# weibohuang0314/pixel_aware_gyro_aided_klt_feature_tracker

Measured on AMD Instinct MI355X. Metric: tracked features/sec (21x21, 3-lvl, 30 iter), higher is better.
Workload: dtype f32 sampling, f64 normal equations; 1 GPU; cfg1_euroc_752x480: 752x480 pair, 1000 keypoints (1000/GPU), gyro-predicted affine init, h=10, L=3, I=30 (synthetic stand-in for BASELINE configs[1]); mode=shard-weak, features_total=1000, features_active=1000, step_mode=graph

## Files before the change

### pixel_aware_gyro_aided_klt_feature_tracker_amd/csrc/pagk_device.h

```cpp
#pragma once
#include <hip/hip_runtime.h>
#include <stdint.h>

namespace pagk {

constexpr int kMaxLevels = 8;

struct DevLevel {
    const uint32_t *quad;
    int cols, rows;
    float fcols, frows;
    float fcols_m1, frows_m1;
};

__device__ __forceinline__ int ld_agent(const int *p) { return __hip_atomic_load(p, __ATOMIC_RELAXED, __HIP_MEMORY_SCOPE_AGENT); }
__device__ __forceinline__ void st_agent(int *p, int v) { __hip_atomic_store(p, v, __ATOMIC_RELAXED, __HIP_MEMORY_SCOPE_AGENT); }

struct SuspState {
    int level;
    int iter;
    float dx, dy, dg, db, lastCost;
    int iters;
};

// ... 481 lines not shown
                                                      uint32_t sv, OperandRange &rg)
{
    const double H00 = M[0][0], H10 = M[1][0], H11 = M[1][1], H20 = M[2][0], H21 = M[2][1], H22 = M[2][2];
    const double H30 = M[3][0], H31 = M[3][1], H32 = M[3][2], H33 = M[3][3];
    const bool recip = (sv & SV_LLT_RECIP) != 0;
    auto scale = [&](double n, const Den &D, double rx) { return recip ? n * rx : div_by<FAST>(n, D, rg); };
    const bool ok0 = FAST || (!(H00 <= 0.0));
    const double d0 = pivot_root_early<FAST>(ok0, H00, H00, rg);
    const Den D0 = den_prepare<FAST>(d0, rg);
    double rx = recip ? div_by<FAST>(1.0, D0, rg) : 0.0;
    const double q10 = scale(H10, D0, rx), q20 = scale(H20, D0, rx), q30 = scale(H30, D0, rx);
    const double r0 = div_by<FAST>(b[0], D0, rg);
    const double L10 = ok0 ? q10 : H10, L20 = ok0 ? q20 : H20, L30 = ok0 ? q30 : H30;
    const double x1 = H11 - L10 * L10;
    const bool ok1 = FAST || (ok0 && !(x1 <= 0.0));
    const double d1 = pivot_root_early<FAST>(ok1, x1, H11, rg);
    const Den D1 = den_prepare<FAST>(d1, rg);
    rx = recip ? div_by<FAST>(1.0, D1, rg) : 0.0;
    const double q21 = scale(H21 - L20 * L10, D1, rx), q31 = scale(H31 - L30 * L10, D1, rx);
    const double r1 = div_by<FAST>(b[1] - L10 * r0, D1, rg);
    const double L21 = ok1 ? q21 : H21, L31 = ok1 ? q31 : H31;
    double s = L20 * L20;
    s += L21 * L21;
    const double x2 = H22 - s;
    const bool ok2 = FAST || (ok1 && !(x2 <= 0.0));
    const double d2 = pivot_root_early<FAST>(ok2, x2, H22, rg);
    const Den D2 = den_prepare<FAST>(d2, rg);
    s = L30 * L20;
    s += L31 * L21;
    rx = recip ? div_by<FAST>(1.0, D2, rg) : 0.0;
    const double q32 = scale(H32 - s, D2, rx);
    const double r2 = div_by<FAST>(b[2] - (L20 * r0 + L21 * r1), D2, rg);
    const double L32 = ok2 ? q32 : H32;
    const double a0 = L30 * L30, a1 = L31 * L31, a2 = L32 * L32;
    const double x3 = H33 - ((sv & SV_PIVOT_TREE) ? a0 + (a1 + a2) : (a0 + a1) + a2);
    const bool ok3 = ok2 && !(x3 <= 0.0);
    const double d3 = pivot_root<FAST>(ok3, x3, H33, rg);
    const Den D3 = den_prepare<FAST>(d3, rg);
    const double c0 = L30 * r0, c1 = L31 * r1, c2 = L32 * r2;
    const double r3 = div_by<FAST, true>(b[3] - ((sv & SV_LOWER_SEQ) ? (c0 + c1) + c2 : c0 + (c1 + c2)), D3, rg);
    return llt4_upper_nsq<FAST>(r0, r1, r2, r3, L10, L20, L21, L30, L31, L32, D0, D1, D2, D3, sv, x, rg);
}

__device__ __forceinline__ double llt4_solve_nsq(const double (&M)[4][4], const double (&b)[4], double (&x)[4],
                                                 uint32_t sv)
{
    OperandRange rg;
    double nsq = llt4_solve_nsq_form<true>(M, b, x, sv, rg);
    if (!rg.in_range()) nsq = llt4_solve_nsq_form<false>(M, b, x, sv, rg);
    return nsq;
}

__device__ __forceinline__ double llt4_solve_norm(const double (&M)[4][4], const double (&b)[4], double (&x)[4],
                                                  uint32_t sv)
{
    OperandRange rg;
    return sqrt(llt4_solve_nsq_form<false>(M, b, x, sv, rg));
}

__device__ __forceinline__ double lane_bcast(double v, int src)
{
    int lo = __double2loint(v), hi = __double2hiint(v);
    lo = __builtin_amdgcn_readlane(lo, src);
    hi = __builtin_amdgcn_readlane(hi, src);
    return __hiloint2double(hi, lo);
}
template <int K>
__device__ __forceinline__ double row_bcast(double v)
{
    return __builtin_amdgcn_update_dpp(0.0, v, 0x150 + K, 0xf, 0xf, false);
}

#ifdef PAGK_COUNT_REDO
static __device__ uint32_t g_redo_lo, g_redo_hi;
#endif
template <int K, bool ROWB>
__device__ __forceinline__ double solve_bcast(double v)
{
    if constexpr (ROWB)
        return row_bcast<K>(v);
    else
        return lane_bcast(v, K);
}
template <bool FAST, bool ROWB = false>
__device__ __forceinline__ double llt4_solve_nsq_lanes_form(const double (&M)[4][4], const double (&b)[4], int l,
                                                            double (&x)[4], uint32_t sv, OperandRange &rg)
{
    const double H00 = M[0][0], H10 = M[1][0], H11 = M[1][1], H20 = M[2][0], H21 = M[2][1], H22 = M[2][2];
    const double H30 = M[3][0], H31 = M[3][1], H32 = M[3][2], H33 = M[3][3];
    const bool recip = (sv & SV_LLT_RECIP) != 0;
    auto column = [&](double n, const Den &D, bool fwd) {
        const double q = div_by<FAST>(n, D, rg);
        if (!recip) return q;
        const double rx = div_by<FAST>(1.0, D, rg);
        return fwd ? q : n * rx;
    };
    const bool ok0 = FAST || (!(H00 <= 0.0));
    const double d0 = pivot_root_early<FAST>(ok0, H00, H00, rg);
    const Den D0 = den_prepare<FAST>(d0, rg);
    const double n0 = l == 0 ? b[0] : (l == 1 ? H10 : (l == 2 ? H20 : H30));
    const double q0 = column(n0, D0, l == 0);
    const double own0 = (l == 0 || ok0) ? q0 : n0;
    double r0 = solve_bcast<0, ROWB>(own0);
    const double L10 = solve_bcast<1, ROWB>(own0), L20 = solve_bcast<2, ROWB>(own0), L30 = solve_bcast<3, ROWB>(own0);
    const double x1 = H11 - L10 * L10;
    const bool ok1 = FAST || (ok0 && !(x1 <= 0.0));
    const double d1 = pivot_root_early<FAST>(ok1, x1, H11, rg);
    const Den D1 = den_prepare<FAST>(d1, rg);
    const double h1 = l == 2 ? H21 : H31;
    const double n1 = l == 1 ? b[1] - L10 * r0 : h1 - (l == 2 ? L20 : L30) * L10;
    const double q1 = column(n1, D1, l == 1);
    const double own1 = (l == 1 || ok1) ? q1 : h1;
    double r1 = solve_bcast<1, ROWB>(own1);
    const double L21 = solve_bcast<2, ROWB>(own1), L31 = solve_bcast<3, ROWB>(own1);
    double s = L20 * L20;
    s += L21 * L21;
    const double x2 = H22 - s;
    const bool ok2 = FAST || (ok1 && !(x2 <= 0.0));
    const double d2 = pivot_root_early<FAST>(ok2, x2, H22, rg);
    const Den D2 = den_prepare<FAST>(d2, rg);
    s = L30 * L20;
    s += L31 * L21;
    const double n2 = l == 2 ? b[2] - (L20 * r0 + L21 * r1) : H32 - s;
    const double q2 = column(n2, D2, l == 2);
    const double own2 = (l == 2 || ok2) ? q2 : H32;
    double r2 = solve_bcast<2, ROWB>(own2);
    const double L32 = solve_bcast<3, ROWB>(own2);
    const double a0 = L30 * L30, a1 = L31 * L31, a2 = L32 * L32;
    const double x3 = H33 - ((sv & SV_PIVOT_TREE) ? a0 + (a1 + a2) : (a0 + a1) + a2);
    const bool ok3 = ok2 && !(x3 <= 0.0);
    const double d3 = pivot_root<FAST>(ok3, x3, H33, rg);
    const Den D3 = den_prepare<FAST>(d3, rg);
    const double c0 = L30 * r0, c1 = L31 * r1, c2 = L32 * r2;
    const double r3 = div_by<FAST, true>(b[3] - ((sv & SV_LOWER_SEQ) ? (c0 + c1) + c2 : c0 + (c1 + c2)), D3, rg);
    return llt4_upper_nsq<FAST>(r0, r1, r2, r3, L10, L20, L21, L30, L31, L32, D0, D1, D2, D3, sv, x, rg);
}

template <bool ROWB = false>
__device__ __forceinline__ double llt4_solve_nsq_lanes(const double (&M)[4][4], const double (&b)[4], int l,
                                                       double (&x)[4], uint32_t sv)
{
    OperandRange rg;
    double nsq = llt4_solve_nsq_lanes_form<true, ROWB>(M, b, l, x, sv, rg);
#ifndef PAGK_EXPERIMENT_NO_REDO
    if (__builtin_amdgcn_ballot_w64(!rg.in_range() && l < 4) != 0) nsq = llt4_solve_nsq_lanes_form<false, ROWB>(M, b, l, x, sv, rg);
#endif
#ifdef PAGK_COUNT_REDO
    g_redo_lo = rg.t;
#endif
    return nsq;
}

__device__ __forceinline__ double repeat_sum_f64(double q, int P)
{
    if (!(q > 0.0)) return (double)P * q;
    double x = 32.0 * q;
    int k = 32;
    double top = __hiloint2double((__double2hiint(q) & 0x7ff00000) + (6 << 20), 0);
    double M = 0.75 * top;
#pragma unroll
    for (int b = 0; b < 5; b++) {
        const double I = (q + M) - M;
        const float est = (float)(top - x) * __builtin_amdgcn_rcpf((float)I);
        int n = (int)est - 1;
        const int lim = (P - k) - 4 * (5 - b);
        n = n > lim ? lim : n;
        n = n < 0 ? 0 : n;
        x = __builtin_fma((double)n, I, x);
        k += n + 4;
        x = x + q;
        x = x + q;
        x = x + q;
        x = x + q;
        M *= 2.0;
        top *= 2.0;
    }
    return x;
}

__device__ __forceinline__ double add_penalty_hb(const TrackArgs &a, float dx, float dy, double (&H)[4][4],
                                                 double (&b)[4])
{
    double d = (double)sqrtf(dx * dx + dy * dy);
    double e_pen = (double)a.lam_invlog * soft_log((double)a.alpha * d + 1);
    double jx = (double)a.lam_invlog_alpha / ((double)a.alpha * d + 1) * ((double)dx / d);
    double jy = (double)a.lam_invlog_alpha / ((double)a.alpha * d + 1) * ((double)dy / d);
    H[0][0] += jx * jx;
    H[1][0] += jy * jx;
    H[1][1] += jy * jy;
    H[2][0] += 0.0 * jx;
    H[2][1] += 0.0 * jy;
    H[2][2] += 0.0 * 0.0;
    H[3][0] += 0.0 * jx;
    H[3][1] += 0.0 * jy;
    H[3][2] += 0.0 * 0.0;
    H[3][3] += 0.0 * 0.0;
    b[0] += jx * e_pen;
    b[1] += jy * e_pen;
    b[2] += 0.0 * e_pen;
    b[3] += 0.0 * e_pen;
    return e_pen * e_pen;
}
__device__ __forceinline__ void add_penalty(const TrackArgs &a, float dx, float dy, double (&H)[4][4],
                                            double (&b)[4], float &cost)
{
    const double epsq = add_penalty_hb(a, dx, dy, H, b);
    cost = (float)((double)cost + epsq);
}

__device__ __forceinline__ void distort_point(const TrackArgs &a, float ux, float uy, float &ox, float &oy)
{
    if (!a.distort_on) {
        ox = ux;
        oy = uy;
        return;
    }
    float x = (ux - a.cx) * a.fx_inv;
    float y = (uy - a.cy) * a.fy_inv;
    float r2 = x * x + y * y;
    float r4 = r2 * r2;
    float r6 = r4 * r2;
    float xd = x * (1 + a.k1 * r2 + a.k2 * r4 + a.k3 * r6) + 2 * a.p1 * x * y + a.p2 * (r2 + 2 * x * x);
    float yd = y * (1 + a.k1 * r2 + a.k2 * r4 + a.k3 * r6) + a.p1 * (r2 + 2 * y * y) + 2 * a.p2 * x * y;
    ox = a.fx * xd + a.cx;
    oy = a.fy * yd + a.cy;
}
// ... 3 lines not shown
```

### pixel_aware_gyro_aided_klt_feature_tracker_amd/csrc/pagk_hip.hip

```cpp
#include <hip/hip_runtime.h>

#include <cmath>
#include <cstdio>
#include <cstdlib>
#include <cstring>
#include <new>
#include <vector>

#include "../../include/pagk.h"
#include "pagk_kernels.h"

using namespace pagk;

namespace {

constexpr int kSlots = 6;
constexpr int kUserSlots = 4;

struct FrameSlot {
    int w = 0, h = 0, L = 0;
    int wrap0 = 1;
    int pad0 = 0;
    uint8_t *u8[kMaxLevels] = {};
    uint32_t *quad[kMaxLevels] = {};
// ... 288 lines not shown
{
    int lw[kMaxLevels], lh[kMaxLevels];
    level_dims(s.w, s.h, s.L, lw, lh);
    bool all_even = s.L <= 4;
    for (int l = 0; l + 1 < s.L; l++) all_even = all_even && !(lw[l] & 1) && !(lh[l] & 1);
    return all_even;
}

int slot_build(pagk_ctx *ctx, FrameSlot &s, const uint8_t *src0, int64_t pitch0, int wrap0)
{
    s.pad0 = wrap0 ? 0 : 2;
    int lw[kMaxLevels], lh[kMaxLevels];
    level_dims(s.w, s.h, s.L, lw, lh);
    dim3 blk(32, 8);
    if (ctx->ev_pyr[0] && !in_capture(ctx)) HIPCHK(ctx, hipEventRecord(ctx->ev_pyr[0], ctx->stream));
    bool all_even = true;
    for (int l = 0; l + 1 < s.L; l++) all_even = all_even && !(lw[l] & 1) && !(lh[l] & 1);
    if (s.L <= 4 && !ctx->unfused_pyramid && all_even) {
        PyrArgs pa;
        const int nb = make_pyr_args(s, src0, pitch0, wrap0, &pa);
        hipLaunchKernelGGL(k_pyramid_fused, dim3(nb), dim3(256), 0, ctx->stream, pa);
        HIPCHK(ctx, hipGetLastError());
        if (ctx->ev_pyr[1] && !in_capture(ctx)) HIPCHK(ctx, hipEventRecord(ctx->ev_pyr[1], ctx->stream));
        if (!in_capture(ctx)) ctx->pyr_timed = true;
        s.wrap0 = wrap0;
        s.valid = true;
        return PAGK_OK;
    }
    const uint8_t *src = src0;
    int64_t pitch = pitch0;
    for (int l = 0; l < s.L; l++) {
        if (l > 0) {
            dim3 grd((lw[l] + 31) / 32, (lh[l] + 7) / 8);
            if (!(lw[l - 1] & 1) && !(lh[l - 1] & 1))
                hipLaunchKernelGGL(k_pyr_down, grd, blk, 0, ctx->stream, src, pitch, lw[l], lh[l], s.u8[l]);
            else
                hipLaunchKernelGGL(k_pyr_down_linear, grd, blk, 0, ctx->stream, src, pitch, lw[l - 1], lh[l - 1], lw[l],
                                   lh[l], 1. / ((double)lw[l] / lw[l - 1]), 1. / ((double)lh[l] / lh[l - 1]), s.u8[l]);
            src = s.u8[l];
            pitch = lw[l];
        }
        dim3 grd((lw[l] + 31) / 32, (lh[l] + 7) / 8);
        hipLaunchKernelGGL(k_build_quads, grd, blk, 0, ctx->stream, src, pitch, lw[l], lh[l], l == 0 ? wrap0 : 1,
                           s.quad[l]);
    }
    HIPCHK(ctx, hipGetLastError());
    if (ctx->ev_pyr[1] && !in_capture(ctx)) HIPCHK(ctx, hipEventRecord(ctx->ev_pyr[1], ctx->stream));
    if (!in_capture(ctx)) ctx->pyr_timed = true;
    s.wrap0 = wrap0;
    s.valid = true;
    return PAGK_OK;
}

int check_params(const pagk_params *p)
{
    if (!p) return PAGK_E_ARG;
    if (p->half_patch < 1 || p->half_patch > PAGK_MAX_HALF_PATCH) return PAGK_E_ARG;
    if (p->iterations < 0 || p->pyramids < 1 || p->pyramids > PAGK_MAX_PYRAMIDS) return PAGK_E_ARG;
    if (p->inverse) return PAGK_E_UNSUPPORTED;
    if (p->solver_variant & ~(SV_LOWER_SEQ | SV_UPPER_TREE | SV_NORM_SEQ | SV_LLT_RECIP | SV_PIVOT_TREE)) return PAGK_E_ARG;
    return PAGK_OK;
}

void fill_level(DevLevel &d, const FrameSlot &s, int l)
{
    int w = s.w, h = s.h;
    for (int k = 0; k < l; k++) {
        w = (int)(w * 0.5);
        h = (int)(h * 0.5);
    }
    d.quad = s.quad[l];
    d.cols = w;
    d.rows = h;
    d.fcols = (float)w;
    d.frows = (float)h;
    d.fcols_m1 = (float)(w - 1);
    d.frows_m1 = (float)(h - 1);
}

int lv_check(pagk_ctx *ctx)
{
    if (ctx->lv_error && *static_cast<volatile int *>(ctx->lv_error) != 0) {
        *static_cast<volatile int *>(ctx->lv_error) = 0;
        snprintf(ctx->err, sizeof(ctx->err), "a wave of the level-by-level tracking launch gave up waiting for the level above");
        return PAGK_E_HIP;
    }
    return PAGK_OK;
}

int no_live_graphs(pagk_ctx *ctx, const char *what)
{
    for (int k = 0; k < pagk_ctx::kGraphs; k++)
        if (ctx->graph_execs[k]) {
            snprintf(ctx->err, sizeof(ctx->err), "%s would have to grow while graph %d of this context is alive (its nodes hold the old "
                     "pointers): destroy the graph first, or run the largest launch once before capturing", what, k);
            return PAGK_E_ARG;
        }
    return PAGK_OK;
}

int quad_capacity(pagk_ctx *ctx, int half)
{
    const int slot = half == 5 ? 0 : (half == 7 ? 1 : 2);
    if (ctx->quad_capacity[slot] == 0) {
        int per_cu = 0;
        hipError_t e = half == 5   ? hipOccupancyMaxActiveBlocksPerMultiprocessor(&per_cu, k_track_quad<2>, 64, 0)
                       : half == 7 ? hipOccupancyMaxActiveBlocksPerMultiprocessor(&per_cu, k_track_quad<4>, 64, 0)
                                   : hipOccupancyMaxActiveBlocksPerMultiprocessor(&per_cu, k_track_quad<7>, 64, 0);
        if (e != hipSuccess || per_cu <= 0) per_cu = 16;
        ctx->quad_capacity[slot] = per_cu * (ctx->cus > 0 ? ctx->cus : 256);
    }
    return ctx->quad_capacity[slot];
}

int quad_budget_for(pagk_ctx *ctx, int waves, int iterations, int levels, int half)
{
    if (ctx->quad_budget >= 0) return ctx->quad_budget;
    if (iterations * levels < 60) return 0;
    const long long cap = quad_capacity(ctx, half);
    const bool exposed_tail = 100ll * waves > 45 * cap && 100ll * waves <= 125 * cap;
    if (ctx->concurrency != 1 || !exposed_tail || (in_capture(ctx) && !ctx->capturing)) return 0;
    return 20;
}

int levels_budget_for(pagk_ctx *ctx, int quads, int iterations, int levels, int half, bool *live)
{
    const bool foreign = in_capture(ctx) && !ctx->capturing;
    *live = !foreign || ctx->quad_budget >= 0;
    if (ctx->quad_budget >= 0) return ctx->quad_budget;
    if (iterations * levels < 60 || ctx->concurrency != 1) return 0;
    const long long cap = quad_capacity(ctx, half);
    if (100ll * quads <= 45 * cap) return 0;
    if (foreign && 100ll * quads > 125 * cap) return 0;
    return 20;
}

void fill_param_args(TrackArgs &a, const pagk_params *p)
{
    a.half = p->half_patch;
    a.iterations = p->iterations;
    a.has_gyro = p->has_gyro_predict_initial;
    a.illum = p->consider_illumination;
    a.use_affine = p->consider_affine;
    a.penalty = p->regularization_penalty;
    a.calc_ncc = p->calculate_ncc;
    a.solver = p->solver_variant;
    float invlog = p->inv_log_max_dist != 0.0f ? p->inv_log_max_dist
                                               : pagk_inv_log_max_dist(p->alpha, p->max_distance);
    a.lam_invlog = p->lambda * invlog;
    a.lam_invlog_alpha = a.lam_invlog * p->alpha;
    a.alpha = p->alpha;
    a.win_size_inv = (double)(1.0f / (2.0f * p->half_patch + 1.0f) / (2.0f * p->half_patch + 1.0f));
    a.distort_on = p->dist_coef[0] != 0.0f;
    a.fx = p->fx, a.fy = p->fy, a.cx = p->cx, a.cy = p->cy;
    a.fx_inv = (float)(1.0 / (double)p->fx);
    a.fy_inv = (float)(1.0 / (double)p->fy);
    a.k1 = p->dist_coef[0], a.k2 = p->dist_coef[1], a.p1 = p->dist_coef[2], a.p2 = p->dist_coef[3];
    a.k3 = p->n_dist_coef == 5 ? p->dist_coef[4] : 0.0f;
}

int launch_track(pagk_ctx *ctx, const pagk_params *p, const FrameSlot &sr, const FrameSlot &sc, int n,
                 const float *d_pt_ref, const float *d_pt_init, const float *d_affine, const uint8_t *d_status,
                 const pagk_outputs *o, const PyrArgs *pyr = nullptr, int pyr_blocks = 0, bool *pyr_done = nullptr)
{
    if (pyr_done) *pyr_done = false;
    TrackArgs a;
    memset(&a, 0, sizeof a);
    a.n_levels = p->pyramids;
    for (int l = 0; l < p->pyramids; l++) {
        fill_level(a.l1[l], sr, l);
        fill_level(a.l2[l], sc, l);
        a.scales[l] = l == 0 ? 1.0f : (float)((double)a.scales[l - 1] * 0.5);
    }
    a.n = n;
    a.pt_ref = d_pt_ref;
    a.pt_init = d_pt_init;
    a.affine = d_affine;
    a.status_in = d_status;
    a.pt_un = o->pt_un;
    a.pt_dist = o->pt_dist;
    a.status = o->status;
    a.pix_err = o->pix_err;
    a.dist_pred = o->dist_pred;
    a.ncc = o->ncc;
    a.iters = o->iters;
#if defined(PAGK_STAMPS) || defined(PAGK_COUNT_REDO) || defined(PAGK_TIC)
    a.dbg = reinterpret_cast<unsigned long long *>(getenv("PAGK_DBG_PTR") ? strtoull(getenv("PAGK_DBG_PTR"), nullptr, 0) : 0ull);
#endif
    fill_param_args(a, p);
    a.prio_k = ctx->prio_k;
    a.prio_stats = ctx->prio_stats;
    a.prio_kbuf = ctx->prio_stats ? reinterpret_cast<const int *>(ctx->prio_stats + 2) : nullptr;

    if (ctx->ev_trk[0] && !in_capture(ctx)) HIPCHK(ctx, hipEventRecord(ctx->ev_trk[0], ctx->stream));
    if (n > 0) {
        const int Pm = (2 * a.half + 1) * (2 * a.half + 1);
        const bool mfma_ok = a.half == 5 || a.half == 7 || a.half == 10;
        ctx->last_handover = false;
        const bool lean = !a.penalty && a.solver == 0;
        const long long n_sel = (long long)n * ctx->concurrency;
#ifdef PAGK_ALL_VARIANTS
        const bool use_rows = mfma_ok && !a.calc_ncc && a.iterations >= 1 && ctx->kernel == 6;
#else
        const bool use_rows = false;
#endif
        const bool use_levels = mfma_ok && !a.calc_ncc && p->pyramids >= 2 && ctx->lv_error &&
                                (ctx->kernel == 7 || (ctx->kernel == 0 && (ctx->concurrency == 1 || ctx->levels_shared) &&
                                                      n_sel >= ctx->levels_min_features));
        const bool quad_like = ctx->kernel == 5 || ctx->kernel == 6 || ctx->kernel == 7;
        const bool use_quad = !use_rows && !use_levels && mfma_ok && !a.calc_ncc && (quad_like || (ctx->kernel == 0 && n_sel >= ctx->quad_min_features));
        const bool use_wave = !use_quad && !use_rows && !use_levels && mfma_ok && (ctx->kernel == 3 || quad_like || (ctx->kernel == 0 && n_sel >= ctx->wave_min_features));
#ifdef PAGK_ALL_VARIANTS
        const bool use_mfma = !use_wave && mfma_ok && (ctx->kernel == 2 || (ctx->kernel == 0 && n_sel >= ctx->mfma_min_features));
#else
        const bool use_mfma = false;
#endif
        ctx->last_variant = ctx->kernel == 1 ? 1 : use_levels ? 7 : use_rows ? 6 : (use_quad ? 5 : (use_wave ? 3 : ((ctx->kernel == 4 && mfma_ok) ? 4 : (use_mfma ? 2 : 0))));
        if (ctx->kernel == 1) {
            hipLaunchKernelGGL(k_track_thread, dim3((n + 63) / 64), dim3(64), 0, ctx->stream, a);
#ifdef PAGK_ALL_VARIANTS
        } else if (use_rows) {
            const int nch = (Pm + 63) / 64;
            const int slot = a.half == 5 ? 0 : (a.half == 7 ? 1 : 2);
            if (ctx->rows_capacity[slot] == 0) {
                int per_cu = 0, cus = 0;
                hipError_t oe = a.half == 5   ? hipOccupancyMaxActiveBlocksPerMultiprocessor(&per_cu, k_track_rows<2>, 64, 0)
                                : a.half == 7 ? hipOccupancyMaxActiveBlocksPerMultiprocessor(&per_cu, k_track_rows<4>, 64, 0)
                                              : hipOccupancyMaxActiveBlocksPerMultiprocessor(&per_cu, k_track_rows<7>, 64, 0);
                HIPCHK(ctx, oe);
                HIPCHK(ctx, hipDeviceGetAttribute(&cus, hipDeviceAttributeMultiprocessorCount, ctx->device));
                ctx->rows_capacity[slot] = per_cu * cus > 0 ? per_cu * cus : 1024;
            }
            int waves = (n + 3) / 4 < ctx->rows_capacity[slot] ? (n + 3) / 4 : ctx->rows_capacity[slot];
            if (ctx->rows_waves_cap > 0 && waves > ctx->rows_waves_cap) waves = ctx->rows_waves_cap;
            const size_t need = (size_t)waves * 4 * nch * 64 * sizeof(float);
            if (need > ctx->quad_ws_bytes) {
                if (in_capture(ctx)) {
                    snprintf(ctx->err, sizeof(ctx->err), "the row kernel's workspace would have to be (re)allocated during graph capture");
                    return PAGK_E_ARG;
                }
                if (int gr = no_live_graphs(ctx, "the row kernel's workspace")) return gr;
                if (ctx->quad_ws) HIPCHK(ctx, hipFree(ctx->quad_ws));
                ctx->quad_ws = nullptr;
                ctx->quad_ws_bytes = 0;
                HIPCHK(ctx, hipMalloc(&ctx->quad_ws, need));
                ctx->quad_ws_bytes = need;
            }
            a.ws = static_cast<float *>(ctx->quad_ws);
            a.queue = static_cast<int *>(ctx->queue);
            HIPCHK(ctx, hipMemsetAsync(a.queue, 0, 4, ctx->stream));
            auto launch = [&](auto kern) -> hipError_t {
                hipLaunchKernelGGL(kern, dim3(waves), dim3(64), 0, ctx->stream, a);
                return hipGetLastError();
            };
            hipError_t e = hipErrorInvalidValue;
            if (a.half == 5) e = launch(k_track_rows<2>);
            else if (a.half == 7) e = launch(k_track_rows<4>);
            else if (a.half == 10) e = launch(k_track_rows<7>);
            HIPCHK(ctx, e);
#endif
        } else if (use_quad || use_levels) {
            const int nch = (Pm + 63) / 64, nq = (n + 3) / 4, waves = use_levels ? nq * p->pyramids : nq;
            const size_t need = (size_t)waves * 4 * nch * 64 * sizeof(float);
            const size_t ready_bytes = use_levels ? align_up((size_t)(p->pyramids - 1) * 8 * ((nq + 7) / 8) * 4, 256) : 0;
            const size_t susp_zero = 256 + align_up((size_t)n * 4, 256);
            const size_t need_lv = use_levels ? 32768 + ready_bytes + susp_zero + (size_t)n * 16 + (size_t)n * sizeof(SuspState) : 0;
            if (need > ctx->quad_ws_bytes || need_lv > ctx->lv_bytes) {
                if (in_capture(ctx)) {
                    snprintf(ctx->err, sizeof(ctx->err), "the quad kernel's workspace would have to be (re)allocated during graph capture");
                    return PAGK_E_ARG;
                }
                if (int gr = no_live_graphs(ctx, "the quad kernel's workspace")) return gr;
                if (need > ctx->quad_ws_bytes) {
                    if (ctx->quad_ws) HIPCHK(ctx, hipFree(ctx->quad_ws));
                    ctx->quad_ws = nullptr;
// ... 1623 lines not shown
```

### pixel_aware_gyro_aided_klt_feature_tracker_amd/csrc/pagk_pipe_kernel.h

```cpp
#pragma once

namespace pagk {


__device__ __forceinline__ bool lds_wait_ge(const int *flag, int want)
{
    for (uint32_t look = 0; look < kPipeWaitLooks; look++) {
        if (__builtin_amdgcn_readfirstlane(*reinterpret_cast<const volatile int *>(flag)) >= want) return true;
        __builtin_amdgcn_s_sleep(1);
    }
    return false;
}

__device__ __forceinline__ void lds_store_b32(uint32_t addr, int v)
{
    asm volatile("ds_write_b32 %0, %1" ::"v"(addr), "v"(v) : "memory");
}

template <int H, bool LEAN>
__device__ __forceinline__ void track_pipe_body(const TrackArgs &a, const int i, const SuspState *resume = nullptr)
{
    static_assert(H >= 8 && H <= 10, "two-round patches only");
    constexpr int kBlock = 256;
    constexpr int Wd = 2 * H + 1, P = Wd * Wd, PP = (P + 31) / 32 * 32, PS = PP + 1;
    constexpr int TAIL = P % 32;
    constexpr bool HAS_B = P > 320, HAS_C = P > 384;
    extern __shared__ __attribute__((aligned(16))) unsigned char lds_raw[];
    const int tid = threadIdx.x;
    const int wave = __builtin_amdgcn_readfirstlane(tid >> 6), lane = tid & 63;

    double *stream = reinterpret_cast<double *>(lds_raw);
    float *esq = reinterpret_cast<float *>(stream + (size_t)8 * PS);
    double *cslot = reinterpret_cast<double *>(esq + PP);
    double *acc = cslot + 2;
    double *sh_upd = acc + 16;
    float *sh_cost = reinterpret_cast<float *>(sh_upd + 5);
    int *flags = reinterpret_cast<int *>(sh_cost + 2 + 2);
    double *h22 = reinterpret_cast<double *>(flags + 4);
    double *sh_pen = h22 + 2;

    const float *init = a.has_gyro ? a.pt_init : a.pt_ref;
    float p2x = init[2 * i], p2y = init[2 * i + 1];
    if (!a.status_in[i]) {
        if (tid == 0) write_outputs(a, i, p2x, p2y, 0, 0.0f, 0, 0.0f, 0);
        return;
    }
    float A00 = 1, A01 = 0, A10 = 0, A11 = 1;
    if (a.use_affine) {
        A00 = a.affine[4 * i], A01 = a.affine[4 * i + 1], A10 = a.affine[4 * i + 2], A11 = a.affine[4 * i + 3];
    }
    const float refx = a.pt_ref[2 * i], refy = a.pt_ref[2 * i + 1];
    if (tid < 4) flags[tid] = 0;

    int pix[3];
    pix[0] = tid;
    pix[1] = (wave == 3 ? 320 : 256) + lane;
    pix[2] = 384 + lane;
    float px[3], py[3], wx[3], wy[3];
#pragma unroll
    for (int r = 0; r < 3; r++) {
        const int p = pix[r] < P ? pix[r] : P - 1;
        const int yy = p / Wd, xx = p - yy * Wd;
        const int x = xx - H, y = yy - H;
        px[r] = (float)x;
        py[r] = (float)y;
        if (a.use_affine) {
            wx[r] = A00 * (float)x + A01 * (float)y;
            wy[r] = A10 * (float)x + A11 * (float)y;
        } else {
            wx[r] = (float)x;
            wy[r] = (float)y;
        }
    }
    const float fh = (float)H;
    const float ext_x = fabsf(A00) * fh + fabsf(A01) * fh + 2.0f;
    const float ext_y = fabsf(A10) * fh + fabsf(A11) * fh + 2.0f;

    const int lr = lane & 15;
    const int cid = wave * 4 + (lane >> 4);
    const uint32_t row_addr = wave < 2 ? lds_off(stream + (size_t)cid * PS) + 16u * lr : lds_off(esq) + 8u * lr;
    const uint32_t flag_addr = lds_off(flags);
    const int acc_slot = wave < 2 ? (lr == 0 ? (cid == 7 ? 9 : cid) : ((lr == 1 && cid >= 5) ? (cid == 7 ? 10 : cid + 2) : -1)) : -1;

    int succ = 1, iters = 0, seq = 0;
    [[maybe_unused]] constexpr bool kPrioByWork = true;
    PAGK_PRIO_DECL
    float lastCost = 0.0f;
#ifdef PAGK_STAMPS
    unsigned long long st[14] = {0, 0, 0, 0, 0, 0, 0, 0, 0, 0, 0, 0, 0, 0};
    unsigned long long t_begin = __builtin_amdgcn_s_memtime(), t0, t1;
    const unsigned long long rt_begin = __builtin_amdgcn_s_memrealtime();
#define STAMP(k)                                  \
    t1 = __builtin_amdgcn_s_memtime();            \
    st[k] += t1 - t0;                             \
    t0 = t1;
#else
#define STAMP(k)
#endif
#if defined(PAGK_TIC) && defined(PAGK_TOC)
    unsigned long long pt_t0 = 0, pt_sum = 0;
#define POINT(k)                                                                   \
    if (wave == 0) {                                                               \
        if ((k) == PAGK_TIC) pt_t0 = __builtin_amdgcn_s_memtime();                 \
        if ((k) == PAGK_TOC) pt_sum += __builtin_amdgcn_s_memtime() - pt_t0;       \
    }
#else
#define POINT(k)
#endif

    const int level_first = resume ? resume->level : a.n_levels - 1;
    for (int level = level_first; level >= 0; level--) {
#ifdef PAGK_STAMPS
        t0 = __builtin_amdgcn_s_memtime();
#endif
        const DevLevel &L1 = a.l1[level];
        const DevLevel L2 = pin_level(a.l2[level]);
        const float ptx = refx * a.scales[level], pty = refy * a.scales[level];
        float nx, ny;
        if (level == a.n_levels - 1) {
            nx = p2x * a.scales[level];
            ny = p2y * a.scales[level];
        } else {
            nx = (float)((double)(p2x * 1.0f) / 0.5);
            ny = (float)((double)(p2y * 1.0f) / 0.5);
        }
        float dx = nx - ptx, dy = ny - pty, dg = 0.0f, db = 0.0f;
        lastCost = 0.0f;
        succ = 1;
        int iter_first = 0;
        if (resume && level == level_first) {
            dx = resume->dx, dy = resume->dy, dg = resume->dg, db = resume->db;
            lastCost = resume->lastCost;
            iters = resume->iters;
            iter_first = resume->iter;
        }

        const float cneg = -sample<true>(L1, ptx, pty);
        const double cd = (double)cneg;
        float s1[3];
        s1[0] = sample<true>(L1, ptx + px[0], pty + py[0]);
        s1[1] = s1[2] = 0.0f;
        if (wave >= 2) {
            s1[1] = sample<true>(L1, ptx + px[1], pty + py[1]);
            if (HAS_C && wave == 2) s1[2] = sample<true>(L1, ptx + px[2], pty + py[2]);
        }
        double row_s1 = 1.0;
        switch (cid) {
            case 3: case 4: row_s1 = -1.0; break;
            case 5: case 6: row_s1 = lr == 0 ? cd : 1.0; break;
            case 7: row_s1 = lr == 0 ? -cd : -1.0; break;
            default: break;
        }
        if (level == level_first && wave == 1) {
            const double s = repeat_sum_f64(cd * cd, P);
            if (lane == 0) h22[level & 1] = s;
        }

        STAMP(0)
        for (int iter = iter_first; iter < a.iterations; iter++) {
            iters++;
            seq++;
            PAGK_PRIO_TIER
            POINT(0)
            const float bx = ptx + dx, by = pty + dy;
            const float gain = 1.0f + dg;
            const bool interior = (bx - ext_x >= 0.0f) & (bx + ext_x < L2.fcols_m1) &
                                  (by - ext_y >= 0.0f) & (by + ext_y < L2.frows_m1);
            auto emit = [&](const FiveTaps &t, int p, float s1v) {
                const Five s = sample5_finish(t);
                if (p < P) {
                    const float e = s.c + db - gain * s1v;
                    const float Ix = 0.5f * (s.xp - s.xm);
                    const float Iy = 0.5f * (s.yp - s.ym);
                    const double dIx = (double)Ix, dIy = (double)Iy, de = (double)e;
                    stream[0 * PS + p] = dIx * dIx;
                    stream[1 * PS + p] = dIy * dIx;
                    stream[2 * PS + p] = dIy * dIy;
                    stream[3 * PS + p] = dIx * de;
                    stream[4 * PS + p] = dIy * de;
                    stream[5 * PS + p] = dIx;
                    stream[6 * PS + p] = dIy;
                    stream[7 * PS + p] = de;
                    esq[p] = e * e;
                }
            };
            if (interior) {
                const FiveTaps t = sample5_issue<false>(L2, bx + wx[0], by + wy[0]);
                emit(t, pix[0], s1[0]);
            } else {
                const FiveTaps t = sample5_issue<true>(L2, bx + wx[0], by + wy[0]);
                emit(t, pix[0], s1[0]);
            }
            __syncthreads();
            STAMP(1)
            POINT(1)
            if (wave < 2) {
                PRIO(PAGK_PRIO_N_CHAIN)
                const uint32_t seq_ab = (uint32_t)__builtin_amdgcn_readfirstlane((HAS_B ? 2 : 1) * seq);
                const uint32_t seq_c = (uint32_t)__builtin_amdgcn_readfirstlane(seq);
                const double s = chain_rows_f64_piped<H>(row_addr, row_s1, flag_addr, seq_ab, seq_c);
                if (acc_slot >= 0) acc[acc_slot] = s;
                if (wave == 1) {
                    lds_store_b32(flag_addr + 8u, seq);
                    STAMP(4)
                    PRIO(PAGK_PRIO_N_REST)
                    if (iter == iter_first && level > 0) {
                        const float nptx = refx * a.scales[level - 1], npty = refy * a.scales[level - 1];
                        const double ncd = (double)(-sample<true>(a.l1[level - 1], nptx, npty));
                        const double s22 = repeat_sum_f64(ncd * ncd, P);
                        if (lane == 0) h22[(level - 1) & 1] = s22;
                    }
                } else {
                    typedef double f64x2 __attribute__((ext_vector_type(2)));
                    f64x2 q0, q1, q2, q3, q4, q5;
                    bool acc_there = false;
                    {
                        int f;
                        const uint32_t fad = flag_addr + 8u, aad = lds_off(acc);
                        for (uint32_t look = 0; look < kPipeWaitLooks; look++) {
                            asm volatile("ds_read_b32 %[f], %[fa]\n\t"
                                         "ds_read_b128 %[q0], %[aa]\n\t"
                                         "ds_read_b128 %[q1], %[aa] offset:16\n\t"
                                         "ds_read_b128 %[q2], %[aa] offset:32\n\t"
                                         "ds_read_b128 %[q3], %[aa] offset:48\n\t"
                                         "ds_read_b128 %[q4], %[aa] offset:64\n\t"
                                         "ds_read_b128 %[q5], %[aa] offset:80\n\t"
                                         "s_waitcnt lgkmcnt(0)"
                                         : [f] "=&v"(f), [q0] "=&v"(q0), [q1] "=&v"(q1), [q2] "=&v"(q2), [q3] "=&v"(q3),
                                           [q4] "=&v"(q4), [q5] "=&v"(q5)
                                         : [fa] "v"(fad), [aa] "v"(aad)
                                         : "memory");
                            if (__builtin_amdgcn_readfirstlane(f) >= seq) {
                                acc_there = true;
                                break;
                            }
                            if (look >= 8) __builtin_amdgcn_s_sleep(1);
                        }
                    }
                    STAMP(2)
                    POINT(2)
                    if (tid < 4) {
                        double Hm[4][4], b[4], upd[4];
                        Hm[0][0] = acc_there ? q0.x : __builtin_nan("");
                        Hm[1][0] = q0.y;
                        Hm[1][1] = q1.x;
                        b[0] = q1.y;
                        b[1] = q2.x;
                        Hm[2][0] = q2.y;
                        Hm[2][1] = q3.x;
                        Hm[3][0] = q3.y;
                        Hm[3][1] = q4.x;
                        b[2] = q4.y;
                        b[3] = q5.x;
                        Hm[2][2] = h22[level & 1];
                        Hm[3][2] = (double)P * cd;
                        Hm[3][3] = (double)P;
                        double epsq = 0.0;
                        if constexpr (!LEAN) {
                            if (a.penalty) epsq = add_penalty_hb(a, dx, dy, Hm, b);
                        }
                        const double unorm = llt4_solve_nsq_lanes<true>(Hm, b, tid, upd, LEAN ? 0u : a.solver);
                        if (tid == 0) {
                            sh_upd[0] = upd[0];
                            sh_upd[1] = upd[1];
                            sh_upd[2] = upd[2];
                            sh_upd[3] = upd[3];
                            sh_upd[4] = unorm;
                            if constexpr (!LEAN) sh_pen[0] = epsq;
                        }
                    }
                    PRIO(PAGK_PRIO_N_REST)
                    POINT(3)
                }
            } else if (wave == 2) {
                PRIO(PAGK_PRIO_N_SAMP)
                auto round1 = [&](auto clamp_tag) {
                    constexpr bool CL = decltype(clamp_tag)::value;
                    const FiveTaps ta = sample5_issue<CL>(L2, bx + wx[1], by + wy[1]);
                    if constexpr (HAS_C) {
                        const FiveTaps tc = sample5_issue<CL>(L2, bx + wx[2], by + wy[2]);
                        emit(ta, pix[1], s1[1]);
                        asm volatile("s_waitcnt lgkmcnt(0)" ::: "memory");
                        if (lane == 0) atomicAdd(flags, 1);
                        STAMP(8)
                        emit(tc, pix[2], s1[2]);
                        asm volatile("s_waitcnt lgkmcnt(0)" ::: "memory");
                        lds_store_b32(flag_addr + 4u, seq);
                        STAMP(9)
                    } else {
                        emit(ta, pix[1], s1[1]);
                        asm volatile("s_waitcnt lgkmcnt(0)" ::: "memory");
                        if (lane == 0) atomicAdd(flags, 1);
                    }
                };
                if (interior)
                    round1(std::false_type{});
                else
                    round1(std::true_type{});
                PRIO(PAGK_PRIO_N_REST)
            } else {
                if constexpr (HAS_B) {
                    PRIO(PAGK_PRIO_N_SAMP)
                    if (interior) {
                        const FiveTaps tb = sample5_issue<false>(L2, bx + wx[1], by + wy[1]);
                        emit(tb, pix[1], s1[1]);
                    } else {
                        const FiveTaps tb = sample5_issue<true>(L2, bx + wx[1], by + wy[1]);
                        emit(tb, pix[1], s1[1]);
                    }
                    asm volatile("s_waitcnt lgkmcnt(0)" ::: "memory");
                    if (lane == 0) atomicAdd(flags, 1);
                    STAMP(10)
                }
                PRIO(PAGK_PRIO_N_COST)
                const float c = chain_rows_f32_piped<H>(row_addr, flag_addr, (uint32_t)__builtin_amdgcn_readfirstlane((HAS_B ? 2 : 1) * seq),
                                                        (uint32_t)__builtin_amdgcn_readfirstlane(seq));
                if (lane == 0) sh_cost[0] = c;
                STAMP(13)
                PRIO(PAGK_PRIO_N_REST)
            }
            __syncthreads();
            STAMP(3)
            POINT(4)
            const double u0 = sh_upd[0], u1 = sh_upd[1], u2 = sh_upd[2], u3 = sh_upd[3], unorm = sh_upd[4];
            float cost = sh_cost[0];
            if constexpr (!LEAN) {
                if (a.penalty) cost = (float)((double)cost + sh_pen[0]);
            }
            if (u0 != u0) {
                succ = 0;
                break;
            }
            if (iter > 0 && cost > lastCost) break;
            dx = (float)((double)dx + u0);
            dy = (float)((double)dy + u1);
            if (a.illum) {
                dg = (float)((double)dg + u2);
                db = (float)((double)db + u3);
            }
            lastCost = cost;
            succ = 1;
            if (unorm < kNormSqConverged) break;
#ifdef PAGK_STAMPS
            asm volatile("" : "+v"(dx), "+v"(dy), "+v"(dg), "+v"(db));
            STAMP(12)
#endif
#if defined(PAGK_TIC) && defined(PAGK_TOC)
            asm volatile("" : "+v"(dx), "+v"(dy), "+v"(dg), "+v"(db));
            POINT(5)
#endif
        }
        p2x = ptx + dx;
        p2y = pty + dy;
    }
    PAGK_PRIO_RESET
    float ncc = 1.0f;
    if (a.calc_ncc) {
        float *vref = reinterpret_cast<float *>(stream), *vcur = vref + PP;
        float *tnum = vcur + PP, *td1 = tnum + PP, *td2 = td1 + PP;
        const DevLevel &R0 = a.l1[0], &C0 = a.l2[0];
        constexpr int nfull = P / 32;
        float vr[2], vc[2];
        __syncthreads();
#pragma unroll
        for (int r = 0; r < 2; r++) {
            int k = tid + kBlock * r;
            k = k < P ? k : P - 1;
            int xi = k / Wd - H, yi = k - (k / Wd) * Wd - H;
            vr[r] = sample<true>(R0, refx + xi, refy + yi);
            if (a.use_affine) {
// ... 74 lines not shown
```

Before: 12.06 million features/s.

## Split normal-equation rows across chain waves so the solve starts before all sums arrive

The mapping of chain rows to the two chain waves is permuted so that wave 0 computes the first Cholesky column's entries (H00, H10, H20, H30, b0) itself and takes them by lane broadcast. Wave 0 then starts the 4x4 LLT solve at once. The remaining sums written by wave 1 are read from LDS late, issued after the first pivot root and waited on only before the second column. The goal is to hide the inter-wave handoff latency behind the first solve column. In exchange it adds a more intricate polling path, a timeout that sets an lv_error flag, and a non-LEAN path that still waits up front.

```diff
diff --git a/pixel_aware_gyro_aided_klt_feature_tracker_amd/csrc/pagk_device.h b/pixel_aware_gyro_aided_klt_feature_tracker_amd/csrc/pagk_device.h
--- a/pixel_aware_gyro_aided_klt_feature_tracker_amd/csrc/pagk_device.h
+++ b/pixel_aware_gyro_aided_klt_feature_tracker_amd/csrc/pagk_device.h
@@ -587,12 +587,17 @@
     else
         return lane_bcast(v, K);
 }
-template <bool FAST, bool ROWB = false>
+struct SolveNoLate {
+    __device__ __forceinline__ void issue() const {}
+    __device__ __forceinline__ void operator()() const {}
+};
+template <bool FAST, bool ROWB = false, class LATE = SolveNoLate>
 __device__ __forceinline__ double llt4_solve_nsq_lanes_form(const double (&M)[4][4], const double (&b)[4], int l,
-                                                            double (&x)[4], uint32_t sv, OperandRange &rg)
-{
-    const double H00 = M[0][0], H10 = M[1][0], H11 = M[1][1], H20 = M[2][0], H21 = M[2][1], H22 = M[2][2];
-    const double H30 = M[3][0], H31 = M[3][1], H32 = M[3][2], H33 = M[3][3];
+                                                            double (&x)[4], uint32_t sv, OperandRange &rg,
+                                                            const LATE &late = LATE{})
+{
+    const double H00 = M[0][0], H10 = M[1][0], H20 = M[2][0], H22 = M[2][2];
+    const double H30 = M[3][0], H32 = M[3][2], H33 = M[3][3];
     const bool recip = (sv & SV_LLT_RECIP) != 0;
     auto column = [&](double n, const Den &D, bool fwd) {
         const double q = div_by<FAST>(n, D, rg);
@@ -602,12 +607,15 @@
     };
     const bool ok0 = FAST || (!(H00 <= 0.0));
     const double d0 = pivot_root_early<FAST>(ok0, H00, H00, rg);
+    late.issue();
     const Den D0 = den_prepare<FAST>(d0, rg);
     const double n0 = l == 0 ? b[0] : (l == 1 ? H10 : (l == 2 ? H20 : H30));
     const double q0 = column(n0, D0, l == 0);
     const double own0 = (l == 0 || ok0) ? q0 : n0;
     double r0 = solve_bcast<0, ROWB>(own0);
     const double L10 = solve_bcast<1, ROWB>(own0), L20 = solve_bcast<2, ROWB>(own0), L30 = solve_bcast<3, ROWB>(own0);
+    late();
+    const double H11 = M[1][1], H21 = M[2][1], H31 = M[3][1];
     const double x1 = H11 - L10 * L10;
     const bool ok1 = FAST || (ok0 && !(x1 <= 0.0));
     const double d1 = pivot_root_early<FAST>(ok1, x1, H11, rg);
@@ -641,12 +649,12 @@
     return llt4_upper_nsq<FAST>(r0, r1, r2, r3, L10, L20, L21, L30, L31, L32, D0, D1, D2, D3, sv, x, rg);
 }
 
-template <bool ROWB = false>
+template <bool ROWB = false, class LATE = SolveNoLate>
 __device__ __forceinline__ double llt4_solve_nsq_lanes(const double (&M)[4][4], const double (&b)[4], int l,
-                                                       double (&x)[4], uint32_t sv)
+                                                       double (&x)[4], uint32_t sv, const LATE &late = LATE{})
 {
     OperandRange rg;
-    double nsq = llt4_solve_nsq_lanes_form<true, ROWB>(M, b, l, x, sv, rg);
+    double nsq = llt4_solve_nsq_lanes_form<true, ROWB>(M, b, l, x, sv, rg, late);
 #ifndef PAGK_EXPERIMENT_NO_REDO
     if (__builtin_amdgcn_ballot_w64(!rg.in_range() && l < 4) != 0) nsq = llt4_solve_nsq_lanes_form<false, ROWB>(M, b, l, x, sv, rg);
 #endif
diff --git a/pixel_aware_gyro_aided_klt_feature_tracker_amd/csrc/pagk_hip.hip b/pixel_aware_gyro_aided_klt_feature_tracker_amd/csrc/pagk_hip.hip
--- a/pixel_aware_gyro_aided_klt_feature_tracker_amd/csrc/pagk_hip.hip
+++ b/pixel_aware_gyro_aided_klt_feature_tracker_amd/csrc/pagk_hip.hip
@@ -394,7 +394,7 @@
 {
     if (ctx->lv_error && *static_cast<volatile int *>(ctx->lv_error) != 0) {
         *static_cast<volatile int *>(ctx->lv_error) = 0;
-        snprintf(ctx->err, sizeof(ctx->err), "a wave of the level-by-level tracking launch gave up waiting for the level above");
+        snprintf(ctx->err, sizeof(ctx->err), "a wave of a tracking launch gave up waiting (for the level above, or for the other chain wave's sums)");
         return PAGK_E_HIP;
     }
     return PAGK_OK;
@@ -503,6 +503,7 @@
     a.prio_k = ctx->prio_k;
     a.prio_stats = ctx->prio_stats;
     a.prio_kbuf = ctx->prio_stats ? reinterpret_cast<const int *>(ctx->prio_stats + 2) : nullptr;
+    a.lv_error = ctx->lv_error_dev;
 
     if (ctx->ev_trk[0] && !in_capture(ctx)) HIPCHK(ctx, hipEventRecord(ctx->ev_trk[0], ctx->stream));
     if (n > 0) {
diff --git a/pixel_aware_gyro_aided_klt_feature_tracker_amd/csrc/pagk_pipe_kernel.h b/pixel_aware_gyro_aided_klt_feature_tracker_amd/csrc/pagk_pipe_kernel.h
--- a/pixel_aware_gyro_aided_klt_feature_tracker_amd/csrc/pagk_pipe_kernel.h
+++ b/pixel_aware_gyro_aided_klt_feature_tracker_amd/csrc/pagk_pipe_kernel.h
@@ -3,16 +3,7 @@
 namespace pagk {
 
 
-__device__ __forceinline__ bool lds_wait_ge(const int *flag, int want)
-{
-    for (uint32_t look = 0; look < kPipeWaitLooks; look++) {
-        if (__builtin_amdgcn_readfirstlane(*reinterpret_cast<const volatile int *>(flag)) >= want) return true;
-        __builtin_amdgcn_s_sleep(1);
-    }
-    return false;
-}
-
-__device__ __forceinline__ void lds_store_b32(uint32_t addr, int v)
+__device__ __forceinline__ void lds_write_b32(uint32_t addr, int v)
 {
     asm volatile("ds_write_b32 %0, %1" ::"v"(addr), "v"(v) : "memory");
 }
@@ -78,9 +69,10 @@
 
     const int lr = lane & 15;
     const int cid = wave * 4 + (lane >> 4);
-    const uint32_t row_addr = wave < 2 ? lds_off(stream + (size_t)cid * PS) + 16u * lr : lds_off(esq) + 8u * lr;
+    const int row_stream = (0x76423510 >> (4 * cid)) & 15;
+    const uint32_t row_addr = wave < 2 ? lds_off(stream + (size_t)row_stream * PS) + 16u * lr : lds_off(esq) + 8u * lr;
     const uint32_t flag_addr = lds_off(flags);
-    const int acc_slot = wave < 2 ? (lr == 0 ? (cid == 7 ? 9 : cid) : ((lr == 1 && cid >= 5) ? (cid == 7 ? 10 : cid + 2) : -1)) : -1;
+    const int acc_slot = wave == 1 ? (lr == 0 ? (cid == 7 ? 4 : cid - 4) : ((lr == 1 && cid >= 6) ? 2 * cid - 9 : -1)) : -1;
 
     int succ = 1, iters = 0, seq = 0;
     [[maybe_unused]] constexpr bool kPrioByWork = true;
@@ -146,8 +138,8 @@
         }
         double row_s1 = 1.0;
         switch (cid) {
-            case 3: case 4: row_s1 = -1.0; break;
-            case 5: case 6: row_s1 = lr == 0 ? cd : 1.0; break;
+            case 3: case 5: row_s1 = -1.0; break;
+            case 2: case 6: row_s1 = lr == 0 ? cd : 1.0; break;
             case 7: row_s1 = lr == 0 ? -cd : -1.0; break;
             default: break;
         }
@@ -199,9 +191,9 @@
                 const uint32_t seq_ab = (uint32_t)__builtin_amdgcn_readfirstlane((HAS_B ? 2 : 1) * seq);
                 const uint32_t seq_c = (uint32_t)__builtin_amdgcn_readfirstlane(seq);
                 const double s = chain_rows_f64_piped<H>(row_addr, row_s1, flag_addr, seq_ab, seq_c);
-                if (acc_slot >= 0) acc[acc_slot] = s;
                 if (wave == 1) {
-                    lds_store_b32(flag_addr + 8u, seq);
+                    if (acc_slot >= 0) acc[acc_slot] = s;
+                    lds_write_b32(flag_addr + 8u, seq);
                     STAMP(4)
                     PRIO(PAGK_PRIO_N_REST)
                     if (iter == iter_first && level > 0) {
@@ -211,55 +203,94 @@
                         if (lane == 0) h22[(level - 1) & 1] = s22;
                     }
                 } else {
+                    const double H00 = lane_bcast(s, 0), H10 = lane_bcast(s, 16), H20 = lane_bcast(s, 32);
+                    const double H30 = lane_bcast(s, 33), B0 = lane_bcast(s, 48);
                     typedef double f64x2 __attribute__((ext_vector_type(2)));
-                    f64x2 q0, q1, q2, q3, q4, q5;
-                    bool acc_there = false;
-                    {
-                        int f;
-                        const uint32_t fad = flag_addr + 8u, aad = lds_off(acc);
-                        for (uint32_t look = 0; look < kPipeWaitLooks; look++) {
-                            asm volatile("ds_read_b32 %[f], %[fa]\n\t"
-                                         "ds_read_b128 %[q0], %[aa]\n\t"
-                                         "ds_read_b128 %[q1], %[aa] offset:16\n\t"
-                                         "ds_read_b128 %[q2], %[aa] offset:32\n\t"
-                                         "ds_read_b128 %[q3], %[aa] offset:48\n\t"
-                                         "ds_read_b128 %[q4], %[aa] offset:64\n\t"
-                                         "ds_read_b128 %[q5], %[aa] offset:80\n\t"
-                                         "s_waitcnt lgkmcnt(0)"
-                                         : [f] "=&v"(f), [q0] "=&v"(q0), [q1] "=&v"(q1), [q2] "=&v"(q2), [q3] "=&v"(q3),
-                                           [q4] "=&v"(q4), [q5] "=&v"(q5)
-                                         : [fa] "v"(fad), [aa] "v"(aad)
-                                         : "memory");
-                            if (__builtin_amdgcn_readfirstlane(f) >= seq) {
-                                acc_there = true;
-                                break;
-                            }
-                            if (look >= 8) __builtin_amdgcn_s_sleep(1);
-                        }
-                    }
                     STAMP(2)
                     POINT(2)
                     if (tid < 4) {
                         double Hm[4][4], b[4], upd[4];
-                        Hm[0][0] = acc_there ? q0.x : __builtin_nan("");
-                        Hm[1][0] = q0.y;
-                        Hm[1][1] = q1.x;
-                        b[0] = q1.y;
-                        b[1] = q2.x;
-                        Hm[2][0] = q2.y;
-                        Hm[2][1] = q3.x;
-                        Hm[3][0] = q3.y;
-                        Hm[3][1] = q4.x;
-                        b[2] = q4.y;
-                        b[3] = q5.x;
+                        Hm[0][0] = H00;
+                        Hm[1][0] = H10;
+                        Hm[2][0] = H20;
+                        Hm[3][0] = H30;
+                        b[0] = B0;
                         Hm[2][2] = h22[level & 1];
                         Hm[3][2] = (double)P * cd;
                         Hm[3][3] = (double)P;
-                        double epsq = 0.0;
-                        if constexpr (!LEAN) {
+                        struct Late {
+                            const TrackArgs &a;
+                            double (&Hm)[4][4];
+                            double (&b)[4];
+                            uint32_t fad, aad;
+                            int seq;
+                            mutable int f;
+                            mutable f64x2 q0, q1, q2;
+                            mutable bool issued, taken;
+                            __device__ __forceinline__ void read(bool wait) const
+                            {
+                                if (wait)
+                                    asm volatile("ds_read_b32 %[f], %[fa]\n\t"
+                                                 "ds_read_b128 %[q0], %[aa]\n\t"
+                                                 "ds_read_b128 %[q1], %[aa] offset:16\n\t"
+                                                 "ds_read_b128 %[q2], %[aa] offset:32\n\t"
+                                                 "s_waitcnt lgkmcnt(0)"
+                                                 : [f] "=&v"(f), [q0] "=&v"(q0), [q1] "=&v"(q1), [q2] "=&v"(q2)
+                                                 : [fa] "v"(fad), [aa] "v"(aad)
+                                                 : "memory");
+                                else
+                                    asm volatile("ds_read_b32 %[f], %[fa]\n\t"
+                                                 "ds_read_b128 %[q0], %[aa]\n\t"
+                                                 "ds_read_b128 %[q1], %[aa] offset:16\n\t"
+                                                 "ds_read_b128 %[q2], %[aa] offset:32"
+                                                 : [f] "=&v"(f), [q0] "=&v"(q0), [q1] "=&v"(q1), [q2] "=&v"(q2)
+                                                 : [fa] "v"(fad), [aa] "v"(aad)
+                                                 : "memory");
+                            }
+                            __device__ __forceinline__ void issue() const
+                            {
+                                if (issued) return;
+                                issued = true;
+                                read(false);
+                            }
+                            __device__ __forceinline__ void operator()() const
+                            {
+                                if (taken) return;
+                                taken = true;
+                                issue();
+                                asm volatile("s_waitcnt lgkmcnt(0)" : "+v"(f), "+v"(q0), "+v"(q1), "+v"(q2) : : "memory");
+                                if (__builtin_amdgcn_readfirstlane(f) < seq) {
+                                    bool there = false;
+                                    for (uint32_t look = 0; look < kPipeWaitLooks; look++) {
+                                        if (look >= 8) __builtin_amdgcn_s_sleep(1);
+                                        read(true);
+                                        if (__builtin_amdgcn_readfirstlane(f) >= seq) {
+                                            there = true;
+                                            break;
+                                        }
+                                    }
+                                    if (!there) {
+                                        if (threadIdx.x == 0 && a.lv_error) st_agent(a.lv_error, 1);
+                                        q0.x = __builtin_nan("");
+                                    }
+                                }
+                                Hm[1][1] = q0.x;
+                                b[1] = q0.y;
+                                Hm[2][1] = q1.x;
+                                Hm[3][1] = q1.y;
+                                b[2] = q2.x;
+                                b[3] = q2.y;
+                            }
+                        };
+                        const Late take_late{a, Hm, b, flag_addr + 8u, lds_off(acc), seq};
+                        double epsq = 0.0, unorm;
+                        if constexpr (LEAN) {
+                            unorm = llt4_solve_nsq_lanes<true>(Hm, b, tid, upd, 0u, take_late);
+                        } else {
+                            take_late();
                             if (a.penalty) epsq = add_penalty_hb(a, dx, dy, Hm, b);
+                            unorm = llt4_solve_nsq_lanes<true>(Hm, b, tid, upd, a.solver);
                         }
-                        const double unorm = llt4_solve_nsq_lanes<true>(Hm, b, tid, upd, LEAN ? 0u : a.solver);
                         if (tid == 0) {
                             sh_upd[0] = upd[0];
                             sh_upd[1] = upd[1];
@@ -285,7 +316,7 @@
                         STAMP(8)
                         emit(tc, pix[2], s1[2]);
                         asm volatile("s_waitcnt lgkmcnt(0)" ::: "memory");
-                        lds_store_b32(flag_addr + 4u, seq);
+                        lds_write_b32(flag_addr + 4u, seq);
                         STAMP(9)
                     } else {
                         emit(ta, pix[1], s1[1]);
```

After: 12.27 million features/s (median of 6 runs). +1.7%, better.
